# liuQuan98/APR

Hardware: AMD Instinct MI355X
Metric: point-cloud pairs/sec (120k-pt KITTI frame, FCGF encode+match+SVD) (higher is better)
Workload: dtype f32

## Files before the change

apr_amd/_lib.py:

```python
from __future__ import annotations

import ctypes as C
import os

import torch

_HERE = os.path.dirname(os.path.abspath(__file__))
LIB_PATH = os.path.join(_HERE, "lib", "libapr_hip.so")

_p = C.c_void_p
_i32, _i64, _u64, _f32, _f64, _sz = C.c_int32, C.c_int64, C.c_uint64, C.c_float, C.c_double, C.c_size_t

class PairDesc(C.Structure):
    _fields_ = [("f0", C.c_void_p), ("n0", C.c_int64), ("f1", C.c_void_p), ("n1", C.c_int64),
                ("xyz0", C.c_void_p), ("xyz1", C.c_void_p), ("seed", C.c_uint64)]


class SpconvDesc(C.Structure):
    _fields_ = [("inp", C.c_void_p), ("ldi", C.c_int64), ("nbr", C.c_void_p), ("n_out", C.c_int64),
                ("K", C.c_int32), ("cin", C.c_int32), ("cout", C.c_int32), ("relu", C.c_int32),
                ("w_packed", C.c_void_p), ("scale", C.c_void_p), ("shift", C.c_void_p),
                ("residual", C.c_void_p), ("ldr", C.c_int64), ("out", C.c_void_p), ("ldo", C.c_int64),
                ("counters", C.c_void_p), ("plist", C.c_void_p), ("prod_scratch", C.c_void_p),
                ("plist_bytes", C.c_int64), ("w_bf3", C.c_void_p),
# ... 99 lines not shown
    "apr_norm_backward_scratch_bytes": (_sz, [_i64, _i32]),
    "apr_norm_backward": (C.c_int, [_p, _i64, _p, _i64, _i64, _i32, _p, _p, _p, _p, _i64, _p, _p, _p, _sz, _p]),
    "apr_bn_train_fwd": (C.c_int, [_p, _i64, _i64, _i32, _p, _p, C.c_float, C.c_float, _p, _p, _p, _i64, _i32, _p, _i64, _p, _p,
                                   _p, _p, _i32, _p, _sz, _p]),
    "apr_bn_train_bwd": (C.c_int, [_p, _i64, _p, _i64, _p, _i64, _i64, _i32, _p, _p, _p, _i32, _p, _i64, _p, _i64, _p, _p,
                                   _p, _i32, _p, _sz, _p]),
    "apr_weights_flip_transpose": (C.c_int, [_p, _i32, _i32, _i32, _i32, _p, _p]),
    "apr_dense_gemm_bf3": (C.c_int, [_p, _i64, _i64, _i32, _i32, _p, _p, _p, _p, _i64, _i32, _p, _i64, _p]),
    "apr_dense_rows_bf3_ok": (_i32, [_i32, _i32]),
    "apr_dense_rows_bf3_route": (_i32, [_i64, _i32, _i32]),
    "apr_dense_rows_bf3": (C.c_int, [_p, _i64, _i64, _i32, _i32, _p, _p, _p, _p, _i64, _i32, _i32, _p, _i64, _p]),
    "apr_dense_gemm_bf3_norm_scratch_bytes": (_sz, [_i64, _i32, _i32]),
    "apr_dense_gemm_bf3_norm_act": (C.c_int, [_p, _i64, _i64, _i32, _i32, _p, _f32, _p, _i64, _i32, _f32, _p, _i64, _p, _i32, _p,
                                              _sz, _p]),
    "apr_weighted_choice_round": (C.c_int64, [_p, _i64, _p, _i64, _i64, _p, _i64, _p, _p, _i32]),
    "apr_instance_norm_act_seg": (C.c_int, [_p, _i64, _i64, _i32, _f32, _p, _i64, _i32, _f32, _p, _i64, _p, _i32, _p, _sz, _p]),
    "apr_affine_act": (C.c_int, [_p, _i64, _i64, _i32, _p, _p, _p, _i64, _i32, _f32, _p, _i64, _p]),
    "apr_act_backward": (C.c_int, [_p, _i64, _p, _i64, _i64, _i32, _i32, _f32, _p, _i64, _p]),
    "apr_l2_normalize": (C.c_int, [_p, _i64, _i64, _i32, _p, _i64, _p]),
    "apr_l2_normalize_backward": (C.c_int, [_p, _i64, _p, _i64, _i64, _i32, _p, _i64, _p]),
    "apr_feature_nn": (C.c_int, [_p, _i64, _p, _i64, _i32, _p, _p]),
    "apr_feature_nn_fast_scratch_bytes": (_sz, [_i64, _i64, _i32]),
    "apr_feature_nn_fast": (C.c_int, [_p, _i64, _p, _i64, _i32, _p, _p, _sz, _p]),
    "apr_nn_unpack": (C.c_int, [_p, _i64, _p, _p, _p]),
    "apr_ransac_scratch_bytes": (_sz, [_i64, _i64]),
    "apr_ransac_pose": (C.c_int, [_p, _i64, _p, _i64, _p, _f64, _f64, _i64, _u64, _p, _sz, _p, _p]),
    "apr_ransac_geometric_scratch_bytes": (_sz, [_i64, _i64, _i64]),
    "apr_ransac_pose_geometric": (C.c_int, [_p, _i64, _p, _i64, _p, _f64, _f64, _i64, _i64, _u64, _p, _sz, _p, _p]),
    "apr_ransac_raw_bytes": (_sz, []),
    "apr_ransac_pose_geometric_async": (C.c_int, [_p, _i64, _p, _i64, _p, _f64, _f64, _i64, _i64, _u64, _p, _sz, _p, _p]),
    "apr_ransac_decode": (C.c_int, [_p, _p]),
    "apr_irls_pose": (C.c_int, [_p, _p, _p, _i64, _p, _p, _sz, _p]),
    "apr_match_pose_batch_scratch_bytes": (_sz, [_i32, _i64, _i64, _i32, _i64]),
    "apr_match_pose_batch": (C.c_int, [_p, _i32, _i32, C.c_double, C.c_double, _i64, _p, _sz, _p, _p]),
    "apr_match_pose_batch_slot_bytes": (_sz, [_i32]),
    "apr_match_pose_set_lanes": (C.c_int, [_i32]),
    "apr_match_pose_batch_enqueue": (C.c_int, [_p, _i32, _i32, C.c_double, C.c_double, _i64, _p, _sz, _p, _p]),
    "apr_match_pose_batch_finish": (C.c_int, [_p, _i32, _i32, C.c_double, C.c_double, _i64, _p, _sz, _p, _p, _p]),
    "apr_irls_scratch_bytes": (_sz, [_i64]),
    "apr_valid_pair": (C.c_int, [_p, _i64, _p, _i64, _p, _p, _i64, _i64, _p, _p, _f32, _p, _i64, _i64, _p, _sz, _p]),
    "apr_valid_pair_scratch_bytes": (_sz, [_i64]),
    "apr_contrastive_reduce": (C.c_int, [_p, _p, _i32, _i32, _p, _p, _p, _p, _p, _p, _p, _i32, _i64, _f32, _f32, _p, _p]),
    "apr_grid_subsample_scratch_bytes": (_sz, [_i64]),
    "apr_grid_subsample": (C.c_int, [_p, _i64, _p, _i32, _f32, _p, _i32, _p, _p, _p, _p, _sz, _p]),
    "apr_grid_subsample_async": (C.c_int, [_p, _i64, _p, _i32, _f32, _p, _i32, _p, _p, _p, _p, _sz, _p]),
    "apr_voxel_down_sample_scratch_bytes": (_sz, [_i64]),
# ... 130 lines not shown
```

apr_amd/csrc/common.h:

```cpp
#pragma once
#include <hip/hip_runtime.h>
#include <stdint.h>
#include <stdio.h>
#include <stdlib.h>
#include <string.h>

#include "../../include/apr_hip.h"

static inline int env_int(const char* name, int dflt) {
  const char* v = getenv(name);
  return v ? atoi(v) : dflt;
}

#define APR_API extern "C" __attribute__((visibility("default")))

void apr_set_error(const char* fmt, ...);

#define APR_CHECK_ARG(cond, ...)      \
  do {                                \
    if (!(cond)) {                    \
      apr_set_error(__VA_ARGS__);     \
      return APR_EINVAL;              \
    }                                 \
  } while (0)
// ... 9 lines not shown

#define APR_LAUNCH_CHECK() APR_HIP(hipGetLastError())

static inline int64_t cdiv64(int64_t a, int64_t b) { return (a + b - 1) / b; }

__host__ __device__ static inline size_t apr_align256(size_t x) { return (x + 255) & ~(size_t)255; }

struct AprArena {
  char* base;
  size_t off = 0;
  explicit AprArena(void* scratch) : base((char*)apr_align256((size_t)scratch)) {}
  template <typename T>
  T* take(size_t count) {
    T* p = base ? (T*)(base + off) : nullptr;
    off += apr_align256(count * sizeof(T));
    return p;
  }
  size_t bytes() const { return off + 256; }
  bool fits(size_t scratch_bytes) const { return scratch_bytes >= bytes(); }
};

int apr_internal_nn_brute(const float* f0, int64_t n0, const float* f1, int64_t n1, int32_t c, uint64_t* best,
                          const unsigned* run_if, void* stream);

int apr_internal_fill(void* ptr, int32_t byte_value, size_t bytes, hipStream_t st);

bool apr_internal_dense_ok(int64_t M, int32_t cin, int32_t cout);
bool apr_internal_dense_rows_route(int64_t M, int32_t cin, int32_t cout);
int apr_internal_dense_gemm(const float* in, int64_t ldi, int64_t M, int32_t cin, int32_t cout, const float* wp,
                            const float* scale, const float* shift, const float* residual, int64_t ldr, int32_t relu,
                            float* out, int64_t ldo, hipStream_t st);

int apr_internal_norm_apply_partials(const float* x, int64_t ldx, int32_t c, const int64_t* seg_row0, const int* seg_blk0,
                                     int32_t nseg, const double* partial, float eps, const float* residual, int64_t ldr,
                                     int32_t act_mode, float negative_slope, float* y, int64_t ldy, hipStream_t st);

#ifdef __HIPCC__
__device__ inline int apr_wave_incl_scan(int x) {
  x += __builtin_amdgcn_update_dpp(0, x, 0x111, 0xf, 0xf, true);
  x += __builtin_amdgcn_update_dpp(0, x, 0x112, 0xf, 0xf, true);
  x += __builtin_amdgcn_update_dpp(0, x, 0x114, 0xf, 0xf, true);
  x += __builtin_amdgcn_update_dpp(0, x, 0x118, 0xf, 0xf, true);
  x += __builtin_amdgcn_update_dpp(0, x, 0x142, 0xa, 0xf, true);
  x += __builtin_amdgcn_update_dpp(0, x, 0x143, 0xc, 0xf, true);
  return x;
}
// ... 83 lines not shown
```

apr_amd/csrc/match_mfma.hip:

```cpp
#include "common.h"

namespace {

typedef float f32x4 __attribute__((ext_vector_type(4)));
typedef float f32x2 __attribute__((ext_vector_type(2)));
typedef __bf16 bf16x8 __attribute__((ext_vector_type(8)));

constexpr float kEpsRel = 1e-4f;
constexpr float kEpsAbs = 5e-5f;

__device__ inline unsigned short to_bf16_rne(float x) {
  unsigned u = __float_as_uint(x);
  u += 0x7FFFu + ((u >> 16) & 1u);
  return (unsigned short)(u >> 16);
}

template <int C>
__global__ void k_nn_prep(const float* __restrict__ f, int64_t n, float len_scale, float row_scale,
                          unsigned short* __restrict__ fb, unsigned short* __restrict__ fl, f32x4* __restrict__ meta,
                          unsigned* __restrict__ u_init, unsigned long long* __restrict__ best_init,
                          unsigned* __restrict__ zero_me) {
  constexpr int LPR = C / 4;
  const int64_t t = (int64_t)blockIdx.x * blockDim.x + threadIdx.x;
  const int64_t row = t / LPR;
// ... 506 lines not shown
  const unsigned shared_cap = (unsigned)shared_capacity(n0);
  constexpr int LPR = C / 4;
  if ((uint64_t)qblocks * 4 * (uint64_t)nchunk * (uint64_t)(chunk / 16) + 64 >= (1ull << 32)) {
    apr_set_error("apr_feature_nn_fast: problem too large for the dense-block ids");
    return APR_EINVAL;
  }
  hipLaunchKernelGGL((k_nn_prep2<C>), dim3((unsigned)cdiv64((n0 + n1) * LPR, 256)), dim3(256), 0, st, f0, n0, f1, n1, qb, ql,
                     qmeta, tb, tl, tmeta, U, best, overflow);
  static const int s_dense_min = env_int("APR_NN_DENSE_MIN", kDenseMin);
  static const int s_bound_div = env_int("APR_NN_BOUND_DIV", 4);
  const dim3 grid((unsigned)qblocks, (unsigned)nchunk);
  hipLaunchKernelGGL((k_nn_mfma<C, false>), grid, dim3(256), 0, st, qb, ql, qmeta, n0, tb, tl, tmeta, n1, (int)chunk, U,
                     cand, cand_count, overflow, shared_list, shared_cap, dense_list, overflow + 2, s_bound_div);
  hipLaunchKernelGGL((k_nn_mfma<C, true>), grid, dim3(256), 0, st, qb, ql, qmeta, n0, tb, tl, tmeta, n1, (int)chunk, U,
                     cand, cand_count, overflow, shared_list, shared_cap, dense_list, overflow + 2, s_dense_min);
  const unsigned nwg = (unsigned)(qblocks * nchunk);
  const unsigned nexact = nwg + 256;
  hipLaunchKernelGGL((k_nn_resolve<C>), dim3(nexact + 1024), dim3(256), 0, st, cand, cand_count, nwg, nexact, shared_list,
                     overflow, shared_cap, dense_list, (int)chunk, (unsigned)(qblocks * 4), f0, n0, f1, n1, best);
  APR_LAUNCH_CHECK();
  return APR_OK;
}

}

APR_API size_t apr_feature_nn_fast_scratch_bytes(int64_t n0, int64_t n1, int32_t c) {
  if (n0 < 0 || n1 < 0 || c <= 0) return 0;
  if (n0 < 1) n0 = 1;
  if (n1 < 1) n1 = 1;
  const size_t qblocks = (size_t)cdiv64(n0, 256);
  const size_t nwaves = 4 * (768 + qblocks);
  const size_t nflag = qblocks * 4 * ((2 * (size_t)n1 + 320) / 16 + 1);
  const size_t nlist = nflag > kDenseListCap ? (size_t)kDenseListCap : nflag;
  const auto al = apr_align256;
  return 2 * al((size_t)n0 * c * 2) + 2 * al((size_t)n1 * c * 2) + al((size_t)n0 * 16) + al((size_t)n1 * 16) +
         al((size_t)n0 * 4) + 256 + al(nwaves * 4) + al(nwaves * kCandWave * 8) +
         al((size_t)shared_capacity(n0) * 8) + al(nflag + 64) + al(nlist * 4 + 64) + 512;
}

APR_API int apr_feature_nn_fast(const float* f0, int64_t n0, const float* f1, int64_t n1, int32_t c, uint64_t* best,
                                void* scratch, size_t scratch_bytes, void* stream) {
  hipStream_t st = (hipStream_t)stream;
  APR_CHECK_ARG(n0 >= 0 && n1 > 0 && n1 < (1ll << 31) && n0 < (1ll << 31), "apr_feature_nn_fast: bad shape");
  APR_CHECK_ARG(c == 32 || c == 64 || c == 128, "apr_feature_nn_fast: c=%d, supported: 32, 64, 128", c);
  APR_CHECK_ARG(n1 < (1ll << 24) - 64, "apr_feature_nn_fast: n1 = %lld, supported below 2^24 - 64 targets", (long long)n1);
  APR_CHECK_ARG(((((uintptr_t)f0) | ((uintptr_t)f1)) & 15) == 0, "apr_feature_nn_fast: 16-byte aligned rows required");
  APR_CHECK_ARG(scratch_bytes >= apr_feature_nn_fast_scratch_bytes(n0, n1, c), "apr_feature_nn_fast: scratch too small");
  if (n0 == 0) return APR_OK;
  unsigned long long* b = (unsigned long long*)best;
  if (c == 32) return run_fast<32>(f0, n0, f1, n1, b, scratch, scratch_bytes, st);
  if (c == 64) return run_fast<64>(f0, n0, f1, n1, b, scratch, scratch_bytes, st);
  return run_fast<128>(f0, n0, f1, n1, b, scratch, scratch_bytes, st);
}
```

apr_amd/csrc/ransac.hip:

```cpp
#include <atomic>
#include <cstring>
#include <map>
#include <mutex>
#include <utility>

#include "common.h"
#include "irls.h"

namespace {

struct Hyp {
  double T[12];
  long long it;
  int inliers;
  int pad;
  double err2;
};

__host__ __device__ inline uint64_t splitmix64(uint64_t z) {
  z = (z ^ (z >> 30)) * 0xBF58476D1CE4E5B9ull;
  z = (z ^ (z >> 27)) * 0x94D049BB133111EBull;
  return z ^ (z >> 31);
}

__host__ __device__ inline uint32_t sample_index(uint64_t seed, uint64_t it, int slot, uint32_t n) {
  uint64_t z = splitmix64(seed + (it * 4ull + (uint64_t)slot + 1ull) * 0x9E3779B97F4A7C15ull);
  return (uint32_t)(((z >> 32) * (uint64_t)n) >> 32);
// ... 1371 lines not shown
APR_API size_t apr_match_pose_batch_slot_bytes(int32_t B) { return B > 0 ? (size_t)B * kSlotBytes : 0; }

APR_API int apr_match_pose_batch_enqueue(const apr_pair_desc* pairs, int32_t B, int32_t c, double max_dist,
                                         double edge_ratio, int64_t max_iter, void* scratch, size_t scratch_bytes,
                                         void* slots_host, void* stream) {
  hipStream_t st = (hipStream_t)stream;
  APR_CHECK_ARG(B > 0 && B <= 4096 && pairs && slots_host, "apr_match_pose_batch: bad arguments");
  APR_CHECK_ARG(max_iter > 0 && max_iter < (1ll << 31) && max_dist > 0 && c > 0, "apr_match_pose_batch: bad parameters");
  int64_t n0_max = 0, n1_max = 0;
  for (int i = 0; i < B; ++i) {
    APR_CHECK_ARG(pairs[i].n0 > 0 && pairs[i].n1 > 0 && pairs[i].n0 < (1ll << 31) && pairs[i].n1 < (1ll << 31),
                  "apr_match_pose_batch: empty point set in pair %d", i);
    n0_max = pairs[i].n0 > n0_max ? pairs[i].n0 : n0_max;
    n1_max = pairs[i].n1 > n1_max ? pairs[i].n1 : n1_max;
  }
  AprArena arena(scratch);
  const BatchScratch L = walk_batch(arena, scratch_bytes, B, n0_max, n1_max, c, max_iter);
  APR_CHECK_ARG(L.lanes >= 1, "apr_match_pose_batch: scratch too small");
  const int nlanes = L.lanes;
  char* const slots = L.slots;
  const int64_t cap = max_iter < kChunk ? max_iter : kChunk;
  const double thr_lt = sqrt_lt_threshold(max_dist);
  const bool fast_nn = (c == 32 || c == 64 || c == 128);
  hipStream_t lane_st[kMaxLanes] = {st};
  struct EventGuard {
    hipEvent_t e = nullptr;
    ~EventGuard() { if (e) (void)hipEventDestroy(e); }
  } fork;
  if (nlanes > 1) {
    SideStreams ss;
    const int rc = side_streams(st, &ss);
    if (rc != APR_OK) return rc;
    APR_HIP(hipEventCreateWithFlags(&fork.e, hipEventDisableTiming));
    APR_HIP(hipEventRecord(fork.e, st));
    for (int l = 1; l < nlanes; ++l) {
      lane_st[l] = ss.s[l - 1];
      APR_HIP(hipStreamWaitEvent(lane_st[l], fork.e, 0));
    }
  }
  int rc = APR_OK;
  for (int i = 0; i < B && rc == APR_OK; ++i) {
    const apr_pair_desc& d = pairs[i];
    const int l = i % nlanes;
    hipStream_t ls = lane_st[l];
    char* lp = L.lane0 + (size_t)l * L.lane_bytes;
    uint64_t* best = (uint64_t*)(lp + L.best_off);
    rc = fast_nn ? apr_feature_nn_fast(d.f0, d.n0, d.f1, d.n1, c, best, lp, L.nn_bytes, ls)
                 : apr_feature_nn(d.f0, d.n0, d.f1, d.n1, c, best, ls);
    if (rc != APR_OK) break;
    int64_t* corr = (int64_t*)(L.corr + (size_t)i * L.corr_each);
    AprArena ra(lp + L.ransac_off);
    RansacScratch r = walk_ransac(ra, d.n0, max_iter);
    r.best = (Hyp*)(slots + (size_t)i * kSlotBytes);
    r.total_valid = (long long*)((char*)r.best + sizeof(Hyp));
    hipLaunchKernelGGL(k_init_best, dim3(1), dim3(128), 0, ls, r.best, r.total_valid, r.maxn2, r.n_valid, counter_words(r));
    launch_pack(r, d.xyz0, d.xyz1, d.n1, (const int64_t*)best, d.n0, ls, corr);
    launch_hypotheses(r, d.n0, max_dist, edge_ratio, 0, max_iter, d.seed, (int)cap, ls, true);
    launch_scoring(r, d.n0, thr_lt, (int)cap, ls);
  }
  if (nlanes > 1) {
    for (int l = 1; l < nlanes; ++l) {
      EventGuard join;
      APR_HIP(hipEventCreateWithFlags(&join.e, hipEventDisableTiming));
      APR_HIP(hipEventRecord(join.e, lane_st[l]));
      APR_HIP(hipStreamWaitEvent(st, join.e, 0));
    }
  }
  if (rc != APR_OK) return rc;
  APR_LAUNCH_CHECK();
  APR_HIP(hipMemcpyAsync(slots_host, slots, (size_t)B * kSlotBytes, hipMemcpyDeviceToHost, st));
  return APR_OK;
// ... 186 lines not shown
```

apr_amd/ops.py:

```python
from __future__ import annotations

import ctypes as C
import os

import numpy as np
import torch

from . import _lib
from ._lib import check, ptr, stream


def _lib_():
    return _lib.load()


def _f32(t, name):
    if not t.is_cuda or t.dtype != torch.float32:
        raise _lib.AprHipError(f"{name}: need a float32 GPU tensor (no CPU fallback), got {t.dtype} on {t.device}")
    return t


def _rows(t, name):
    _f32(t, name)
    if t.dim() != 2 or (t.shape[1] > 1 and t.stride(1) != 1):
# ... 1030 lines not shown
    f1 = _f32(f1, "feature_nn.f1").contiguous()
    if f0.shape[1] != f1.shape[1]:
        raise _lib.AprHipError("feature_nn: channel mismatch")
    n0, c = f0.shape
    n1 = f1.shape[0]
    lib = _lib_()
    best = torch.empty(n0, dtype=torch.int64, device=f0.device)
    if impl is None:
        impl = os.environ.get("APR_NN_IMPL", "fast")
    if impl not in ("brute", "fast"):
        raise _lib.AprHipError(f"feature_nn: unknown impl {impl!r}")
    if impl == "fast" and c in (32, 64, 128):
        sb = int(lib.apr_feature_nn_fast_scratch_bytes(n0, n1, c))
        scratch = torch.empty(sb, dtype=torch.uint8, device=f0.device)
        check(lib.apr_feature_nn_fast(ptr(f0), n0, ptr(f1), n1, c, ptr(best), ptr(scratch), sb, stream()))
    else:
        check(lib.apr_feature_nn(ptr(f0), n0, ptr(f1), n1, c, ptr(best), stream()))
    idx = torch.empty(n0, dtype=torch.int64, device=f0.device)
    d2 = torch.empty(n0, dtype=torch.float32, device=f0.device) if return_distance else None
    check(lib.apr_nn_unpack(ptr(best), n0, ptr(idx), ptr(d2), stream()))
    return (idx, d2) if return_distance else idx



def _dev(t, dtype, name):
    if not torch.is_tensor(t) or not t.is_cuda or t.dtype != dtype:
        raise _lib.AprHipError(f"{name}: need a {dtype} GPU tensor (no CPU fallback), got "
                               f"{getattr(t, 'dtype', type(t))} on {getattr(t, 'device', 'the host')}")
    return t.contiguous()


def overlap_labels(correspondence, n_src, n_tgt):
    corr = _dev(correspondence, torch.int64, "overlap_labels.correspondence")
    dev = corr.device
    gt = torch.empty(n_src + n_tgt, dtype=torch.float32, device=dev)
    src_idx = torch.empty(n_src, dtype=torch.int32, device=dev)
    tgt_idx = torch.empty(n_tgt, dtype=torch.int32, device=dev)
    counts = torch.empty(3, dtype=torch.int32, device=dev)
    check(_lib_().apr_overlap_labels(ptr(corr), corr.shape[0], n_src, n_tgt, ptr(gt), ptr(src_idx), ptr(tgt_idx), ptr(counts),
                                     stream()))
    return gt, src_idx, tgt_idx, counts


def weighted_bce(pred, gt, n_dev=None):
    pred, gt = _dev(pred, torch.float32, "weighted_bce.pred"), _dev(gt, torch.float32, "weighted_bce.gt")
    if pred.dim() != 1 or pred.shape != gt.shape:
# ... 699 lines not shown
```

include/apr_hip.h:

```cpp
#ifndef APR_HIP_H
#define APR_HIP_H

#include <stddef.h>
#include <stdint.h>

#ifdef __cplusplus
extern "C" {
#endif

#define APR_OK 0
#define APR_EINVAL (-1)
#define APR_EHIP (-2)
#define APR_ETIMEOUT (-3)
#define APR_ERANGE (-3)

const char* apr_last_error(void);
int apr_version(void);
int apr_device_count(void);
int32_t apr_struct_sizes(int32_t* out, int32_t n);
int apr_event_wait(void* event, int32_t poll_us);
int apr_event_wait_timeout(void* event, int32_t poll_us, int64_t timeout_us);


int64_t apr_hash_capacity(int64_t n);
// ... 228 lines not shown
int apr_ransac_pose_geometric_async(const float* xyz0, int64_t n0, const float* xyz1, int64_t n1,
                                    const int64_t* corr, double max_dist, double edge_ratio, int64_t max_iter,
                                    int64_t max_validation, uint64_t seed, void* scratch, size_t scratch_bytes,
                                    void* raw_dev, void* stream);
int apr_ransac_decode(const void* raw_host, double* result_host);

typedef struct {
  const float* f0; int64_t n0;
  const float* f1; int64_t n1;
  const float* xyz0;
  const float* xyz1;
  uint64_t seed;
} apr_pair_desc;
size_t apr_match_pose_batch_scratch_bytes(int32_t B, int64_t n0_max, int64_t n1_max, int32_t c, int64_t max_iter);
int apr_match_pose_batch(const apr_pair_desc* pairs, int32_t B, int32_t c, double max_dist, double edge_ratio,
                         int64_t max_iter, void* scratch, size_t scratch_bytes, double* results_host, void* stream);
size_t apr_match_pose_batch_slot_bytes(int32_t B);
int apr_match_pose_batch_enqueue(const apr_pair_desc* pairs, int32_t B, int32_t c, double max_dist, double edge_ratio,
                                 int64_t max_iter, void* scratch, size_t scratch_bytes, void* slots_host, void* stream);
int apr_match_pose_batch_finish(const apr_pair_desc* pairs, int32_t B, int32_t c, double max_dist, double edge_ratio,
                                int64_t max_iter, void* scratch, size_t scratch_bytes, const void* slots_host,
                                double* results_host, void* stream);

int apr_ransac_set_screen(int32_t mode);
int apr_ransac_set_option(int32_t option, int32_t value);
int apr_ransac_sampling_launches(int64_t* out2);

int apr_match_pose_set_lanes(int32_t lanes);

int apr_irls_pose(const float* pts0, const float* pts1, const float* weight, int64_t n,
                  float* T_host, void* scratch, size_t scratch_bytes, void* stream);
size_t apr_irls_scratch_bytes(int64_t n);

#define APR_VALID_RECORD_FLOATS 24
int apr_valid_pair(const float* xyz0, int64_t n0, const float* xyz1, int64_t n1, const int64_t* sel0,
                   const int64_t* sel1, int64_t m0, int64_t m1, const int64_t* nn, const float* T_gt,
                   float hit_thresh, float* records, int64_t n_slots, int64_t slot, void* scratch,
                   size_t scratch_bytes, void* stream);
size_t apr_valid_pair_scratch_bytes(int64_t m0);

int apr_contrastive_reduce(const float* pos_f0, const float* pos_f1, int32_t p, int32_t c,
                           const uint64_t* nn01, const uint64_t* nn10, const int64_t* sel0, const int64_t* sel1,
                           const int64_t* pos_ind0, const int64_t* pos_ind1, const int64_t* sorted_pos_keys,
                           int32_t n_keys, int64_t hash_seed, float pos_thresh, float neg_thresh,
                           double* out6, void* stream);

// ... 244 lines not shown
```

Measured before the change: 2756.

## Batch feature nearest-neighbour search across pairs with a two-pass MFMA bound sweep

Adds a batched feature-NN path that packs up to eight pairs into single prep, sweep and resolve launches. The sweep runs a bound pass, then a refine pass that emits candidate lists, which are resolved exactly in fp32, with a brute-force fallback when the lists overflow. The match+pose batch uses this path when there are enough query blocks, instead of running one chunked NN call per pair on the lane streams. This aims to cut per-pair launch overhead and fill the GPU better, at the cost of more scratch memory and more complex overflow handling.

Result: slower. 2722 (-1.2%).

```diff
diff --git a/apr_amd/_lib.py b/apr_amd/_lib.py
--- a/apr_amd/_lib.py
+++ b/apr_amd/_lib.py
@@ -145,6 +145,10 @@
     "apr_feature_nn": (C.c_int, [_p, _i64, _p, _i64, _i32, _p, _p]),
     "apr_feature_nn_fast_scratch_bytes": (_sz, [_i64, _i64, _i32]),
     "apr_feature_nn_fast": (C.c_int, [_p, _i64, _p, _i64, _i32, _p, _p, _sz, _p]),
+    "apr_feature_nn_batch_scratch_bytes": (_sz, [_i32, _i64, _i64, _i32]),
+    "apr_feature_nn_batch_carve_bytes": (_sz, [_p, _i32, _i32]),
+    "apr_feature_nn_batch": (C.c_int, [_p, _i32, _i32, _p, _p, _sz, _p]),
+    "apr_nn_set_option": (C.c_int, [_i32, _i32]),
     "apr_nn_unpack": (C.c_int, [_p, _i64, _p, _p, _p]),
     "apr_ransac_scratch_bytes": (_sz, [_i64, _i64]),
     "apr_ransac_pose": (C.c_int, [_p, _i64, _p, _i64, _p, _f64, _f64, _i64, _u64, _p, _sz, _p, _p]),
diff --git a/apr_amd/csrc/common.h b/apr_amd/csrc/common.h
--- a/apr_amd/csrc/common.h
+++ b/apr_amd/csrc/common.h
@@ -55,6 +55,10 @@
 
 int apr_internal_nn_brute(const float* f0, int64_t n0, const float* f1, int64_t n1, int32_t c, uint64_t* best,
                           const unsigned* run_if, void* stream);
+
+bool apr_internal_nn_batch_wanted(const apr_pair_desc* pairs, int32_t B, int32_t c);
+int apr_internal_nn_sweep(const apr_pair_desc* pairs, int32_t B, int32_t c, uint64_t* const* best, void* scratch,
+                          size_t scratch_bytes, void* stream);
 
 int apr_internal_fill(void* ptr, int32_t byte_value, size_t bytes, hipStream_t st);
 
diff --git a/apr_amd/csrc/match_mfma.hip b/apr_amd/csrc/match_mfma.hip
--- a/apr_amd/csrc/match_mfma.hip
+++ b/apr_amd/csrc/match_mfma.hip
@@ -1,3 +1,5 @@
+#include <atomic>
+
 #include "common.h"
 
 namespace {
@@ -552,6 +554,545 @@
   return APR_OK;
 }
 
+
+constexpr int kNnMaxPairs = 8;
+constexpr int kSweepCandWave = 8192;
+constexpr int kResolveSplit = 4;
+constexpr int kResolveShared = 64;
+constexpr int kResolveDense = 256;
+
+struct NnPairSlot {
+  const float *f0, *f1;
+  unsigned short *qb, *ql, *tb, *tl;
+  f32x4 *qmeta, *tmeta;
+  unsigned* ctl;
+  unsigned* cand_count;
+  unsigned long long* cand;
+  unsigned long long* shared_list;
+  unsigned* dense_list;
+  unsigned long long* best;
+  int n0, n1;
+  unsigned shared_cap, dense_cap;
+  int chunk, bound_len;
+  int qb0, prep0, res0;
+};
+struct NnTable {
+  NnPairSlot p[kNnMaxPairs];
+  int npairs, cand_wave, dense_min;
+};
+
+template <int C>
+__global__ void k_nn_prep_b(NnTable tab) {
+  constexpr int LPR = C / 4;
+  int p = 0;
+  while (p + 1 < tab.npairs && (int)blockIdx.x >= tab.p[p + 1].prep0) ++p;
+  const NnPairSlot& s = tab.p[p];
+  const int64_t n0 = s.n0, n1 = s.n1;
+  const int64_t t = (int64_t)((int)blockIdx.x - s.prep0) * 256 + threadIdx.x;
+  const int64_t row_all = t / LPR;
+  const int g = (int)(t - row_all * LPR);
+  const bool is_q = row_all < n0;
+  const int64_t row = is_q ? row_all : row_all - n0;
+  const int64_t n = is_q ? n0 : n1;
+  const float* f = is_q ? s.f0 : s.f1;
+  const float row_scale = is_q ? -2.0f : 1.0f, len_scale = is_q ? kEpsRel : 1.0f;
+  unsigned short* fb = is_q ? s.qb : s.tb;
+  unsigned short* fl = is_q ? s.ql : s.tl;
+  f32x4* meta = is_q ? s.qmeta : s.tmeta;
+  float sq = 0.f;
+  if (row < n) {
+    f32x4 v = *reinterpret_cast<const f32x4*>(f + row * C + g * 4);
+    sq = v[0] * v[0] + v[1] * v[1] + v[2] * v[2] + v[3] * v[3];
+    v *= row_scale;
+    ushort4 o, ol;
+    o.x = to_bf16_rne(v[0]); o.y = to_bf16_rne(v[1]); o.z = to_bf16_rne(v[2]); o.w = to_bf16_rne(v[3]);
+    ol.x = to_bf16_rne(v[0] - __uint_as_float((unsigned)o.x << 16));
+    ol.y = to_bf16_rne(v[1] - __uint_as_float((unsigned)o.y << 16));
+    ol.z = to_bf16_rne(v[2] - __uint_as_float((unsigned)o.z << 16));
+    ol.w = to_bf16_rne(v[3] - __uint_as_float((unsigned)o.w << 16));
+    *reinterpret_cast<ushort4*>(fb + row * C + g * 4) = o;
+    *reinterpret_cast<ushort4*>(fl + row * C + g * 4) = ol;
+  }
+#pragma unroll
+  for (int d = 1; d < LPR; d <<= 1) sq += __shfl_xor(sq, d);
+  float tlen = 0.f;
+  if (row < n && g == 0) {
+    const float nn = sq;
+    const float sl = kEpsAbs * nn;
+    const float len = sqrtf(nn);
+    meta[row] = (f32x4){len_scale * len, nn + sl, nn - sl, 0.f};
+    if (is_q) s.best[row] = ~0ull; else tlen = len;
+  }
+#pragma unroll
+  for (int d = 32; d >= 1; d >>= 1) tlen = fmaxf(tlen, __shfl_xor(tlen, d));
+  if ((threadIdx.x & 63) == 0 && tlen > 0.f) atomicMax(&s.ctl[3], __float_as_uint(tlen));
+}
+
+struct SweepBound { static constexpr bool refine = false; };
+struct SweepRefine { static constexpr bool refine = true; };
+
+template <int C>
+__global__ __launch_bounds__(256, 2) void k_nn_sweep(NnTable tab) {
+  constexpr int KS = C / 32, QT = 4, TR = C >= 128 ? 32 : 64, NT = TR / 16;
+  constexpr int LPT = (TR * C * 2) / 16 / 256;
+  __shared__ __attribute__((aligned(16))) unsigned short s_h[2][TR * C];
+  __shared__ __attribute__((aligned(16))) unsigned short s_l[2][TR * C];
+  __shared__ f32x4 s_m[2][TR];
+  __shared__ unsigned s_cand[4 * kCandBuf];
+  __shared__ unsigned s_dl[4 * kDlBuf];
+  __shared__ unsigned s_dn[4], s_dbase;
+  int p = 0;
+  while (p + 1 < tab.npairs && (int)blockIdx.x >= tab.p[p + 1].qb0) ++p;
+  const NnPairSlot& s = tab.p[p];
+  const unsigned qblk = blockIdx.x - (unsigned)s.qb0;
+  const int64_t n0 = s.n0, n1 = s.n1;
+  const unsigned short* __restrict__ qb = s.qb;
+  const unsigned short* __restrict__ ql = s.ql;
+  const unsigned short* __restrict__ tb = s.tb;
+  const unsigned short* __restrict__ tl = s.tl;
+  const f32x4* __restrict__ qmeta = s.qmeta;
+  const f32x4* __restrict__ tmeta = s.tmeta;
+  unsigned* const ctl = s.ctl;
+  unsigned long long* const shared_list = s.shared_list;
+  unsigned* const dense_list = s.dense_list;
+  const unsigned shared_cap = s.shared_cap, dense_cap = s.dense_cap;
+  const unsigned cand_wave = (unsigned)tab.cand_wave;
+  const int dense_min = tab.dense_min;
+  const unsigned ntiles = (unsigned)((n1 + 15) >> 4);
+  const int tid = threadIdx.x, lane = tid & 63, wave = tid >> 6;
+  const int l16 = lane & 15, lq = lane >> 4;
+  const int64_t q0 = (int64_t)qblk * 256 + wave * 64;
+  const bool wave_live = q0 < n0;
+  const unsigned wave_id = qblk * 4 + wave;
+  unsigned long long* const my_region = s.cand + (size_t)wave_id * cand_wave;
+  const float len_max = __uint_as_float(ctl[3]);
+  bf16x8 a[QT][KS], al[QT][KS];
+  float thr[QT][4], mn[QT][4];
+#pragma unroll
+  for (int qt = 0; qt < QT; ++qt) {
+    int64_t ra = q0 + qt * 16 + l16;
+    if (ra >= n0) ra = n0 - 1;
+#pragma unroll
+    for (int ks = 0; ks < KS; ++ks) {
+      a[qt][ks] = *reinterpret_cast<const bf16x8*>(qb + ra * C + ks * 32 + lq * 8);
+      al[qt][ks] = *reinterpret_cast<const bf16x8*>(ql + ra * C + ks * 32 + lq * 8);
+    }
+#pragma unroll
+    for (int r = 0; r < 4; ++r) {
+      mn[qt][r] = __builtin_inff();
+      thr[qt][r] = -__builtin_inff();
+    }
+  }
+  int ncand = 0, ndl = 0;
+  unsigned* my_dl = s_dl + wave * kDlBuf;
+  unsigned* my_cand = s_cand + wave * kCandBuf;
+  unsigned flushed = 0;
+
+  auto flush = [&]() {
+    if (ncand == 0) return;
+    auto entry = [&](int e) {
+      const unsigned c = my_cand[e];
+      return ((unsigned long long)(qblk * 256u + (c >> 24)) << 32) | (unsigned long long)(c & 0xffffffu);
+    };
+    if (flushed + ncand <= cand_wave) {
+      unsigned long long* dst = my_region + flushed;
+      for (int e = lane; e < ncand; e += 64) dst[e] = entry(e);
+      flushed += ncand;
+    } else {
+      unsigned base = 0;
+      if (lane == 0) base = atomicAdd(&ctl[1], (unsigned)ncand);
+      base = __shfl(base, 0);
+      if (base + (unsigned)ncand <= shared_cap) {
+        for (int e = lane; e < ncand; e += 64) shared_list[base + e] = entry(e);
+      } else if (lane == 0) {
+        ctl[0] = 1u;
+      }
+    }
+    ncand = 0;
+  };
+
+  uint4 rh[LPT], rl[LPT];
+  f32x4 rm;
+  auto fetch = [&](int64_t jt) {
+#pragma unroll
+    for (int u = 0; u < LPT; ++u) {
+      const int e = u * 256 + tid;
+      int64_t j = jt + (e * 8) / C;
+      if (j >= n1) j = n1 - 1;
+      const int64_t off = j * C + (e * 8) % C;
+      rh[u] = *reinterpret_cast<const uint4*>(tb + off);
+      rl[u] = *reinterpret_cast<const uint4*>(tl + off);
+    }
+    if (tid < TR) {
+      const int64_t j = jt + tid;
+      rm = tmeta[j < n1 ? j : n1 - 1];
+      if (j >= n1) {
+        rm[1] = __builtin_inff();
+        rm[2] = __builtin_inff();
+      }
+    }
+  };
+  auto commit = [&](int buf) {
+#pragma unroll
+    for (int u = 0; u < LPT; ++u) {
+      const int e = u * 256 + tid;
+      const int row = (e * 8) / C, kc = ((e * 8) % C) / 8;
+      const int at = (((kc >> 2) * TR + row) * 4 + (kc & 3)) * 8;
+      *reinterpret_cast<uint4*>(&s_h[buf][at]) = rh[u];
+      *reinterpret_cast<uint4*>(&s_l[buf][at]) = rl[u];
+    }
+    if (tid < TR) s_m[buf][tid] = rm;
+  };
+
+  auto sweep = [&](auto mode, int64_t chunk, int64_t blen) {
+    constexpr bool REFINE = decltype(mode)::refine;
+    int64_t c0 = 0, jt = 0;
+    fetch(0);
+    commit(0);
+    __builtin_amdgcn_s_waitcnt(0x0f70);
+    __syncthreads();
+    int buf = 0;
+    while (true) {
+      int64_t nj = jt + TR, nc0 = c0;
+      if (nj >= min((long long)(c0 + blen), (long long)n1)) {
+        nc0 = c0 + chunk;
+        nj = nc0;
+      }
+      const bool more = nj < n1;
+      if (more) fetch(nj);
+      if (wave_live) {
+        constexpr int NS = C >= 128 ? 1 : 2;
+        bf16x8 b[NS][KS], bl[NS][KS];
+        f32x4 tm[NS];
+        auto frag = [&](int slot, int tt) {
+#pragma unroll
+          for (int ks = 0; ks < KS; ++ks) {
+            b[slot][ks] = *reinterpret_cast<const bf16x8*>(&s_h[buf][((ks * TR + tt * 16 + l16) * 4 + lq) * 8]);
+            bl[slot][ks] = *reinterpret_cast<const bf16x8*>(&s_l[buf][((ks * TR + tt * 16 + l16) * 4 + lq) * 8]);
+          }
+          tm[slot] = s_m[buf][tt * 16 + l16];
+        };
+        frag(0, 0);
+#pragma unroll NS == 2 ? NT : 1
+        for (int tt = 0; tt < NT; ++tt) {
+          if (jt + tt * 16 >= n1) break;
+          const int cur = NS == 2 ? (tt & 1) : 0;
+          if (NS == 2 && tt + 1 < NT) frag(cur ^ 1, tt + 1);
+          if (NS == 1 && tt > 0) frag(0, tt);
+          const float cc = REFINE ? tm[cur][2] : tm[cur][1];
+          const f32x4 cinit = {cc, cc, cc, cc};
+          f32x4 acc[QT];
+#pragma unroll
+          for (int qt = 0; qt < QT; ++qt)
+            acc[qt] = __builtin_amdgcn_mfma_f32_16x16x32_bf16(al[qt][0], b[cur][0], cinit, 0, 0, 0);
+#pragma unroll
+          for (int qt = 0; qt < QT; ++qt)
+            acc[qt] = __builtin_amdgcn_mfma_f32_16x16x32_bf16(a[qt][0], bl[cur][0], acc[qt], 0, 0, 0);
+#pragma unroll
+          for (int ks = 1; ks < KS; ++ks) {
+#pragma unroll
+            for (int qt = 0; qt < QT; ++qt)
+              acc[qt] = __builtin_amdgcn_mfma_f32_16x16x32_bf16(al[qt][ks], b[cur][ks], acc[qt], 0, 0, 0);
+#pragma unroll
+            for (int qt = 0; qt < QT; ++qt)
+              acc[qt] = __builtin_amdgcn_mfma_f32_16x16x32_bf16(a[qt][ks], bl[cur][ks], acc[qt], 0, 0, 0);
+          }
+#pragma unroll
+          for (int ks = 0; ks < KS; ++ks)
+#pragma unroll
+            for (int qt = 0; qt < QT; ++qt)
+              acc[qt] = __builtin_amdgcn_mfma_f32_16x16x32_bf16(a[qt][ks], b[cur][ks], acc[qt], 0, 0, 0);
+          if (!REFINE) {
+#pragma unroll
+            for (int qt = 0; qt < QT; ++qt)
+#pragma unroll
+              for (int r = 0; r < 4; ++r)
+                mn[qt][r] = acc[qt][r] < mn[qt][r] ? acc[qt][r] : mn[qt][r];
+          } else {
+            unsigned cmask = 0;
+#pragma unroll
+            for (int qt = 0; qt < QT; ++qt)
+#pragma unroll
+              for (int r = 0; r < 4; ++r)
+                if (acc[qt][r] <= thr[qt][r]) cmask |= 1u << (qt * 4 + r);
+            if (__any(cmask != 0)) {
+              if (ncand > kCandBuf - 1024) flush();
+              const int c = __popc(cmask);
+              const int incl = apr_wave_incl_scan(c);
+              const int total = __builtin_amdgcn_readlane(incl, 63);
+              if (total >= dense_min) {
+                if (ndl == kDlBuf) {
+                  unsigned base = 0;
+                  if (lane == 0) base = atomicAdd(&ctl[2], (unsigned)ndl);
+                  base = __builtin_amdgcn_readfirstlane(base);
+                  for (int e = lane; e < ndl; e += 64) {
+                    if (base + e < dense_cap) dense_list[base + e] = my_dl[e]; else ctl[0] = 1u;
+                  }
+                  ndl = 0;
+                }
+                if (lane == 0) my_dl[ndl] = wave_id * ntiles + (unsigned)(jt >> 4) + tt;
+                ++ndl;
+                continue;
+              }
+              int pos = ncand + incl - c;
+              const unsigned j = (unsigned)jt + tt * 16 + l16;
+              while (cmask) {
+                const int e = __ffs((int)cmask) - 1;
+                cmask &= cmask - 1;
+                const unsigned i = wave * 64 + (e >> 2) * 16 + lq * 4 + (e & 3);
+                my_cand[pos++] = (i << 24) | j;
+              }
+              ncand += total;
+            }
+          }
+        }
+      }
+      if (more) commit(buf ^ 1);
+      __syncthreads();
+      if (!more) break;
+      jt = nj;
+      c0 = nc0;
+      buf ^= 1;
+    }
+  };
+
+  sweep(SweepBound{}, (int64_t)s.chunk, (int64_t)s.bound_len);
+#pragma unroll
+  for (int qt = 0; qt < QT; ++qt)
+#pragma unroll
+    for (int r = 0; r < 4; ++r) {
+      float v = mn[qt][r];
+#pragma unroll
+      for (int d = 1; d < 16; d <<= 1) v = fminf(v, __shfl_xor(v, d));
+      const int64_t row = q0 + qt * 16 + lq * 4 + r;
+      const bool live = row < n0;
+      const f32x4 m = qmeta[live ? row : n0 - 1];
+      const float u = fmaxf(v + m[1] + m[0] * len_max, 0.f);
+      thr[qt][r] = live ? u - m[2] + m[0] * len_max : -__builtin_inff();
+    }
+  sweep(SweepRefine{}, (int64_t)1 << 40, (int64_t)1 << 40);
+
+  flush();
+  if (lane == 0) {
+    s.cand_count[wave_id] = flushed;
+    s_dn[wave] = (unsigned)ndl;
+  }
+  __syncthreads();
+  if (tid == 0) {
+    const unsigned total = s_dn[0] + s_dn[1] + s_dn[2] + s_dn[3];
+    s_dbase = total ? atomicAdd(&ctl[2], total) : 0u;
+  }
+  __syncthreads();
+  unsigned base = s_dbase;
+  for (int w = 0; w < wave; ++w) base += s_dn[w];
+  for (int e = lane; e < ndl; e += 64) {
+    if (base + e < dense_cap) dense_list[base + e] = my_dl[e]; else ctl[0] = 1u;
+  }
+}
+
+template <int C>
+__global__ __launch_bounds__(256) void k_nn_resolve_b(NnTable tab, int nblocks) {
+  __shared__ __attribute__((aligned(16))) float s_t[4][16 * C];
+  int p = 0;
+  while (p + 1 < tab.npairs && (int)blockIdx.x >= tab.p[p + 1].res0) ++p;
+  const NnPairSlot& s = tab.p[p];
+  const unsigned lb = blockIdx.x - (unsigned)s.res0;
+  const unsigned pair_blocks = (unsigned)((p + 1 < tab.npairs ? tab.p[p + 1].res0 : nblocks) - s.res0);
+  const int64_t n0 = s.n0, n1 = s.n1;
+  const float* __restrict__ f0 = s.f0;
+  const float* __restrict__ f1 = s.f1;
+  unsigned long long* __restrict__ best = s.best;
+  const unsigned* ctl = s.ctl;
+  const int lane = threadIdx.x & 63;
+  const int wave = __builtin_amdgcn_readfirstlane(threadIdx.x >> 6);
+  const unsigned qwaves = (unsigned)((n0 + 255) >> 8) * 4u;
+  if (ctl[0] != 0u) {
+    const int64_t nqt = (n0 + 63) >> 6, ntt = (n1 + 15) >> 4;
+    const int64_t nw = (int64_t)pair_blocks * 4;
+    const int64_t slices = nw / nqt > 0 ? nw / nqt : 1;
+    const int64_t tps = (ntt + slices - 1) / slices;
+    for (int64_t w = (int64_t)lb * 4 + wave; w < nqt * slices; w += nw) {
+      const int64_t q = (w % nqt) * 64 + lane;
+      const int64_t tt0 = (w / nqt) * tps, tt1 = min((long long)(tt0 + tps), (long long)ntt);
+      const float* x = f0 + (q < n0 ? q : n0 - 1) * C;
+      f32x4 xv[C / 4];
+#pragma unroll
+      for (int g = 0; g < C / 4; ++g) xv[g] = *reinterpret_cast<const f32x4*>(x + g * 4);
+      float bd = __builtin_inff();
+      int bj = 0x7fffffff;
+      for (int64_t tt = tt0; tt < tt1; ++tt)
+        nn_tile_eval<C>(s_t[wave], xv, f1, tt * 16, min((long long)(tt * 16 + 16), (long long)n1), lane, bd, bj);
+      if (q < n0 && bj != 0x7fffffff) {
+        const unsigned long long mine = ((unsigned long long)__float_as_uint(bd) << 32) | (unsigned)bj;
+        if (mine < __builtin_nontemporal_load(&best[q])) atomicMin(&best[q], mine);
+      }
+    }
+    return;
+  }
+  const unsigned nregion = qwaves * kResolveSplit, nexact = nregion + kResolveShared;
+  if (lb < nexact) {
+    const bool shared = lb >= nregion;
+    const unsigned region = lb / kResolveSplit;
+    const unsigned n = shared ? min(ctl[1], s.shared_cap) : min(s.cand_count[region], (unsigned)tab.cand_wave);
+    const unsigned long long* src = shared ? s.shared_list : s.cand + (size_t)region * (unsigned)tab.cand_wave;
+    const unsigned first = (shared ? lb - nregion : lb % kResolveSplit) * 256u + threadIdx.x;
+    const unsigned step = (shared ? kResolveShared : kResolveSplit) * 256u;
+    for (unsigned t = first; t < n; t += step) {
+      const unsigned long long ij = src[t];
+      const int64_t i = (int64_t)(ij >> 32), j = (int64_t)(ij & 0xffffffffull);
+      const float* x = f0 + i * C;
+      const float* y = f1 + j * C;
+      float s0 = 0.f, s1 = 0.f, s2 = 0.f, s3 = 0.f;
+#pragma unroll
+      for (int g = 0; g < C / 4; ++g) {
+        const f32x4 xv = *reinterpret_cast<const f32x4*>(x + g * 4);
+        const f32x4 yv = *reinterpret_cast<const f32x4*>(y + g * 4);
+        const float d0 = xv[0] - yv[0], d1 = xv[1] - yv[1], d2 = xv[2] - yv[2], d3 = xv[3] - yv[3];
+        s0 = fmaf(d0, d0, s0);
+        s1 = fmaf(d1, d1, s1);
+        s2 = fmaf(d2, d2, s2);
+        s3 = fmaf(d3, d3, s3);
+      }
+      const float d = (s0 + s1) + (s2 + s3);
+      const unsigned long long mine = ((unsigned long long)__float_as_uint(d) << 32) | (unsigned)j;
+      if (mine < __builtin_nontemporal_load(&best[i])) atomicMin(&best[i], mine);
+    }
+    return;
+  }
+  const unsigned ntiles = (unsigned)((n1 + 15) >> 4);
+  const unsigned n = min(ctl[2], s.dense_cap);
+  const unsigned nwaves = (pair_blocks - nexact) * 4;
+  for (unsigned e = (lb - nexact) * 4 + wave; e < n; e += nwaves) {
+    const unsigned fb = __builtin_amdgcn_readfirstlane(s.dense_list[e]);
+    const unsigned wave_id = fb / ntiles, tile = fb % ntiles;
+    const int64_t q = (int64_t)wave_id * 64 + lane;
+    const int64_t j0 = (int64_t)tile * 16;
+    const int64_t j1 = min((long long)(j0 + 16), (long long)n1);
+    const float* x = f0 + (q < n0 ? q : n0 - 1) * C;
+    f32x4 xv[C / 4];
+#pragma unroll
+    for (int g = 0; g < C / 4; ++g) xv[g] = *reinterpret_cast<const f32x4*>(x + g * 4);
+    float bd = __builtin_inff();
+    int bj = 0x7fffffff;
+    nn_tile_eval<C>(s_t[wave], xv, f1, j0, j1, lane, bd, bj);
+    if (q < n0 && bj != 0x7fffffff) {
+      const unsigned long long mine = ((unsigned long long)__float_as_uint(bd) << 32) | (unsigned)bj;
+      if (mine < __builtin_nontemporal_load(&best[q])) atomicMin(&best[q], mine);
+    }
+  }
+}
+
+enum { kNnOptBatch = 0, kNnOptCandWave = 1, kNnOptDenseCap = 2, kNnOptN = 3 };
+std::atomic<int> g_nn_opt[kNnOptN] = {{-2}, {-2}, {-2}};
+
+int nn_option(int o) {
+  static const int s_env[kNnOptN] = {env_int("APR_NN_BATCH", -1), env_int("APR_NN_CAND_WAVE", 0),
+                                     env_int("APR_NN_DENSE_CAP", 0)};
+  const int v = g_nn_opt[o].load(std::memory_order_relaxed);
+  return v == -2 ? s_env[o] : v;
+}
+int sweep_cand_wave() {
+  const int v = nn_option(kNnOptCandWave);
+  return v > 0 && v < kSweepCandWave ? v : kSweepCandWave;
+}
+unsigned sweep_dense_cap() {
+  const int v = nn_option(kNnOptDenseCap);
+  return v > 0 && (unsigned)v < kDenseListCap ? (unsigned)v : kDenseListCap;
+}
+
+void walk_sweep_pair(AprArena& a, NnPairSlot* slot, int64_t n0, int64_t n1, int c, int cand_wave, unsigned dense_cap) {
+  const size_t qwaves = (size_t)cdiv64(n0, 256) * 4;
+  uint64_t ndense = (uint64_t)qwaves * (uint64_t)cdiv64(n1, 16);
+  if (ndense > dense_cap) ndense = dense_cap;
+  NnPairSlot t;
+  NnPairSlot& s = slot ? *slot : t;
+  s.qb = a.take<unsigned short>((size_t)n0 * c);
+  s.ql = a.take<unsigned short>((size_t)n0 * c);
+  s.tb = a.take<unsigned short>((size_t)n1 * c);
+  s.tl = a.take<unsigned short>((size_t)n1 * c);
+  s.qmeta = a.take<f32x4>(n0);
+  s.tmeta = a.take<f32x4>(n1);
+  s.cand_count = a.take<unsigned>(qwaves);
+  s.cand = a.take<unsigned long long>(qwaves * (size_t)cand_wave);
+  s.shared_list = a.take<unsigned long long>(shared_capacity(n0));
+  s.dense_list = a.take<unsigned>((size_t)ndense + 16);
+  s.shared_cap = (unsigned)shared_capacity(n0);
+  s.dense_cap = (unsigned)ndense;
+}
+
+template <int C>
+int run_sweep(const apr_pair_desc* pairs, int32_t B, uint64_t* const* best, void* scratch, size_t scratch_bytes,
+              hipStream_t st) {
+  static const int s_dense_min = env_int("APR_NN_DENSE_MIN", kDenseMin);
+  static const int s_bound_div = env_int("APR_NN_BOUND_DIV", 4);
+  const int cand_wave = sweep_cand_wave();
+  const unsigned dense_cap = sweep_dense_cap();
+  AprArena a(scratch);
+  unsigned* ctl = a.take<unsigned>((size_t)B * 64);
+  if ((size_t)B * 256 + 256 > scratch_bytes) {
+    apr_set_error("apr_feature_nn_batch: scratch too small");
+    return APR_EINVAL;
+  }
+  int rc = apr_internal_fill(ctl, 0, (size_t)B * 256, st);
+  if (rc != APR_OK) return rc;
+  constexpr int LPR = C / 4;
+  const int ngroups = (int)cdiv64(B, kNnMaxPairs), per = (int)cdiv64(B, ngroups);
+  for (int g0 = 0; g0 < B; g0 += per) {
+    NnTable tab;
+    memset(&tab, 0, sizeof(tab));
+    tab.cand_wave = cand_wave;
+    tab.dense_min = s_dense_min;
+    int np = 0, qb = 0, prep = 0, res = 0;
+    for (int i = g0; i < B && i < g0 + per; ++i) {
+      const apr_pair_desc& d = pairs[i];
+      if (d.n0 == 0) continue;
+      NnPairSlot& s = tab.p[np++];
+      walk_sweep_pair(a, &s, d.n0, d.n1, C, cand_wave, dense_cap);
+      s.f0 = d.f0;
+      s.f1 = d.f1;
+      s.n0 = (int)d.n0;
+      s.n1 = (int)d.n1;
+      s.ctl = ctl + (size_t)i * 64;
+      s.best = (unsigned long long*)best[i];
+      int64_t qblocks, chunk, nchunk;
+      nn_grid(d.n0, d.n1, C, &qblocks, &chunk, &nchunk);
+      s.chunk = (int)chunk;
+      s.bound_len = (int)((chunk / (s_bound_div > 0 ? s_bound_div : 1) + 63) / 64 * 64);
+      s.qb0 = qb;
+      s.prep0 = prep;
+      s.res0 = res;
+      qb += (int)qblocks;
+      prep += (int)cdiv64((d.n0 + d.n1) * LPR, 256);
+      res += (int)qblocks * 4 * kResolveSplit + kResolveShared + kResolveDense;
+    }
+    if (!a.fits(scratch_bytes)) {
+      apr_set_error("apr_feature_nn_batch: scratch too small");
+      return APR_EINVAL;
+    }
+    if (np == 0) continue;
+    tab.npairs = np;
+    hipLaunchKernelGGL((k_nn_prep_b<C>), dim3((unsigned)prep), dim3(256), 0, st, tab);
+    hipLaunchKernelGGL((k_nn_sweep<C>), dim3((unsigned)qb), dim3(256), 0, st, tab);
+    hipLaunchKernelGGL((k_nn_resolve_b<C>), dim3((unsigned)res), dim3(256), 0, st, tab, res);
+  }
+  APR_LAUNCH_CHECK();
+  return APR_OK;
+}
+
+int check_batch_args(const apr_pair_desc* pairs, int32_t B, int32_t c, const char* who) {
+  APR_CHECK_ARG(B > 0 && B <= 4096 && pairs, "%s: bad arguments", who);
+  APR_CHECK_ARG(c == 32 || c == 64 || c == 128, "%s: c=%d, supported: 32, 64, 128", who, c);
+  for (int i = 0; i < B; ++i) {
+    const apr_pair_desc& d = pairs[i];
+    APR_CHECK_ARG(d.n0 >= 0 && d.n1 > 0 && d.n0 < (1ll << 31), "%s: bad shape in pair %d", who, i);
+    APR_CHECK_ARG(d.n1 < (1ll << 24) - 64, "%s: n1 = %lld, supported below 2^24 - 64 targets", who, (long long)d.n1);
+    APR_CHECK_ARG(((((uintptr_t)d.f0) | ((uintptr_t)d.f1)) & 15) == 0, "%s: 16-byte aligned rows required", who);
+    APR_CHECK_ARG((uint64_t)cdiv64(d.n0, 256) * 4 * (uint64_t)cdiv64(d.n1, 16) < (1ull << 32),
+                  "%s: pair %d too large for the dense-block ids", who, i);
+  }
+  return APR_OK;
+}
+
 }
 
 APR_API size_t apr_feature_nn_fast_scratch_bytes(int64_t n0, int64_t n1, int32_t c) {
@@ -582,3 +1123,76 @@
   if (c == 64) return run_fast<64>(f0, n0, f1, n1, b, scratch, scratch_bytes, st);
   return run_fast<128>(f0, n0, f1, n1, b, scratch, scratch_bytes, st);
 }
+
+APR_API size_t apr_feature_nn_batch_carve_bytes(const apr_pair_desc* pairs, int32_t B, int32_t c) {
+  if (!pairs || B <= 0 || !(c == 32 || c == 64 || c == 128)) return 0;
+  AprArena a(nullptr);
+  a.take<unsigned>((size_t)B * 64);
+  const int cand_wave = sweep_cand_wave();
+  const unsigned dense_cap = sweep_dense_cap();
+  for (int i = 0; i < B; ++i) {
+    if (pairs[i].n0 < 0 || pairs[i].n1 <= 0) return 0;
+    if (pairs[i].n0 > 0) walk_sweep_pair(a, nullptr, pairs[i].n0, pairs[i].n1, c, cand_wave, dense_cap);
+  }
+  return a.bytes();
+}
+
+APR_API size_t apr_feature_nn_batch_scratch_bytes(int32_t B, int64_t n0_max, int64_t n1_max, int32_t c) {
+  if (B <= 0 || n0_max < 0 || n1_max < 0 || !(c == 32 || c == 64 || c == 128)) return 0;
+  if (n0_max < 1) n0_max = 1;
+  if (n1_max < 1) n1_max = 1;
+  AprArena a(nullptr);
+  a.take<unsigned>((size_t)B * 64);
+  for (int i = 0; i < B; ++i) walk_sweep_pair(a, nullptr, n0_max, n1_max, c, kSweepCandWave, kDenseListCap);
+  const size_t chunked = apr_feature_nn_fast_scratch_bytes(n0_max, n1_max, c);
+  return a.bytes() > chunked ? a.bytes() : chunked;
+}
+
+bool apr_internal_nn_batch_wanted(const apr_pair_desc* pairs, int32_t B, int32_t c) {
+  static const int s_min_qblocks = env_int("APR_NN_BATCH_MIN_QBLOCKS", 192);
+  const int mode = nn_option(kNnOptBatch);
+  if (mode == 0 || !(c == 32 || c == 64 || c == 128) || B <= 0) return false;
+  int64_t qblocks = 0;
+  for (int i = 0; i < B; ++i) {
+    if (pairs[i].n1 <= 0 || pairs[i].n1 >= (1ll << 24) - 64 || pairs[i].n0 < 0) return false;
+    qblocks += cdiv64(pairs[i].n0, 256);
+  }
+  if (qblocks == 0) return false;
+  return mode == 1 || qblocks / cdiv64(B, kNnMaxPairs) >= s_min_qblocks;
+}
+
+int apr_internal_nn_sweep(const apr_pair_desc* pairs, int32_t B, int32_t c, uint64_t* const* best, void* scratch,
+                          size_t scratch_bytes, void* stream) {
+  const int rc = check_batch_args(pairs, B, c, "apr_feature_nn_batch");
+  if (rc != APR_OK) return rc;
+  hipStream_t st = (hipStream_t)stream;
+  if (c == 32) return run_sweep<32>(pairs, B, best, scratch, scratch_bytes, st);
+  if (c == 64) return run_sweep<64>(pairs, B, best, scratch, scratch_bytes, st);
+  return run_sweep<128>(pairs, B, best, scratch, scratch_bytes, st);
+}
+
+APR_API int apr_feature_nn_batch(const apr_pair_desc* pairs, int32_t B, int32_t c, uint64_t* const* best, void* scratch,
+                                 size_t scratch_bytes, void* stream) {
+  const int rc = check_batch_args(pairs, B, c, "apr_feature_nn_batch");
+  if (rc != APR_OK) return rc;
+  APR_CHECK_ARG(best != nullptr, "apr_feature_nn_batch: NULL best");
+  if (apr_internal_nn_batch_wanted(pairs, B, c)) {
+    if (apr_feature_nn_batch_carve_bytes(pairs, B, c) <= scratch_bytes)
+      return apr_internal_nn_sweep(pairs, B, c, best, scratch, scratch_bytes, stream);
+    APR_CHECK_ARG(nn_option(kNnOptBatch) != 1, "apr_feature_nn_batch: scratch too small for the forced sweep form");
+  }
+  for (int i = 0; i < B; ++i) {
+    const int r = apr_feature_nn_fast(pairs[i].f0, pairs[i].n0, pairs[i].f1, pairs[i].n1, c, best[i], scratch,
+                                      scratch_bytes, stream);
+    if (r != APR_OK) return r;
+  }
+  return APR_OK;
+}
+
+APR_API int apr_nn_set_option(int32_t option, int32_t value) {
+  APR_CHECK_ARG(option >= 0 && option < kNnOptN, "apr_nn_set_option: option 0 .. 2");
+  APR_CHECK_ARG(option == kNnOptBatch ? (value >= -1 && value <= 1) : value >= -1,
+                "apr_nn_set_option: value out of range");
+  g_nn_opt[option].store(value == -1 ? -2 : value, std::memory_order_relaxed);
+  return APR_OK;
+}
diff --git a/apr_amd/csrc/ransac.hip b/apr_amd/csrc/ransac.hip
--- a/apr_amd/csrc/ransac.hip
+++ b/apr_amd/csrc/ransac.hip
@@ -3,6 +3,7 @@
 #include <map>
 #include <mutex>
 #include <utility>
+#include <vector>
 
 #include "common.h"
 #include "irls.h"
@@ -1420,6 +1421,24 @@
   const int64_t cap = max_iter < kChunk ? max_iter : kChunk;
   const double thr_lt = sqrt_lt_threshold(max_dist);
   const bool fast_nn = (c == 32 || c == 64 || c == 128);
+  const size_t best_each = apr_align256((size_t)n0_max * 8);
+  bool nn_batched = false;
+  if (fast_nn && apr_internal_nn_batch_wanted(pairs, B, c)) {
+    const size_t area = (size_t)nlanes * L.lane_bytes, bests = (size_t)B * best_each;
+    nn_batched = bests <= L.nn_bytes && apr_feature_nn_batch_carve_bytes(pairs, B, c) <= area - bests;
+    if (nn_batched) {
+      uint64_t* ptrs[64];
+      std::vector<uint64_t*> many;
+      uint64_t** bp = ptrs;
+      if (B > 64) {
+        many.resize(B);
+        bp = many.data();
+      }
+      for (int i = 0; i < B; ++i) bp[i] = (uint64_t*)(L.lane0 + (size_t)i * best_each);
+      const int rc_nn = apr_internal_nn_sweep(pairs, B, c, bp, L.lane0 + bests, area - bests, st);
+      if (rc_nn != APR_OK) return rc_nn;
+    }
+  }
   hipStream_t lane_st[kMaxLanes] = {st};
   struct EventGuard {
     hipEvent_t e = nullptr;
@@ -1442,9 +1461,10 @@
     const int l = i % nlanes;
     hipStream_t ls = lane_st[l];
     char* lp = L.lane0 + (size_t)l * L.lane_bytes;
-    uint64_t* best = (uint64_t*)(lp + L.best_off);
-    rc = fast_nn ? apr_feature_nn_fast(d.f0, d.n0, d.f1, d.n1, c, best, lp, L.nn_bytes, ls)
-                 : apr_feature_nn(d.f0, d.n0, d.f1, d.n1, c, best, ls);
+    uint64_t* best = nn_batched ? (uint64_t*)(L.lane0 + (size_t)i * best_each) : (uint64_t*)(lp + L.best_off);
+    if (!nn_batched)
+      rc = fast_nn ? apr_feature_nn_fast(d.f0, d.n0, d.f1, d.n1, c, best, lp, L.nn_bytes, ls)
+                   : apr_feature_nn(d.f0, d.n0, d.f1, d.n1, c, best, ls);
     if (rc != APR_OK) break;
     int64_t* corr = (int64_t*)(L.corr + (size_t)i * L.corr_each);
     AprArena ra(lp + L.ransac_off);
diff --git a/apr_amd/ops.py b/apr_amd/ops.py
--- a/apr_amd/ops.py
+++ b/apr_amd/ops.py
@@ -1076,6 +1076,51 @@
     return (idx, d2) if return_distance else idx
 
 
+def feature_nn_batch(feats0, feats1, return_distance=False):
+    B = len(feats0)
+    if B == 0 or B != len(feats1):
+        raise _lib.AprHipError("feature_nn_batch: need the same (non-zero) number of entries in both lists")
+    lib = _lib_()
+    descs = (_lib.PairDesc * B)()
+    keep, bests = [], []
+    c = feats0[0].shape[1]
+    n0m = n1m = 0
+    for i in range(B):
+        f0 = _f32(feats0[i], "feature_nn_batch.feats0").contiguous()
+        f1 = _f32(feats1[i], "feature_nn_batch.feats1").contiguous()
+        if f0.shape[1] != c or f1.shape[1] != c:
+            raise _lib.AprHipError("feature_nn_batch: channel mismatch in pair %d" % i)
+        keep += [f0, f1]
+        d = descs[i]
+        d.f0, d.n0, d.f1, d.n1 = f0.data_ptr(), f0.shape[0], f1.data_ptr(), f1.shape[0]
+        n0m, n1m = max(n0m, f0.shape[0]), max(n1m, f1.shape[0])
+        bests.append(torch.empty(f0.shape[0], dtype=torch.int64, device=f0.device))
+    sb = int(lib.apr_feature_nn_batch_scratch_bytes(B, n0m, n1m, c))
+    if sb == 0:
+        raise _lib.AprHipError("feature_nn_batch: C = %d, supported: 32, 64, 128" % c)
+    scratch = torch.empty(sb, dtype=torch.uint8, device=keep[0].device)
+    bp = (C.c_void_p * B)(*[b.data_ptr() for b in bests])
+    check(lib.apr_feature_nn_batch(descs, B, c, bp, ptr(scratch), sb, stream()))
+    out = []
+    for i in range(B):
+        n0 = descs[i].n0
+        idx = torch.empty(n0, dtype=torch.int64, device=bests[i].device)
+        d2 = torch.empty(n0, dtype=torch.float32, device=bests[i].device) if return_distance else None
+        if n0:
+            check(lib.apr_nn_unpack(ptr(bests[i]), n0, ptr(idx), ptr(d2), stream()))
+        out.append((idx, d2) if return_distance else idx)
+    return out
+
+
+def set_nn_batch(mode):
+    check(_lib_().apr_nn_set_option(0, -1 if mode is None else int(bool(mode))))
+
+
+def set_nn_caps(cand_wave=None, dense=None):
+    check(_lib_().apr_nn_set_option(1, -1 if cand_wave is None else int(cand_wave)))
+    check(_lib_().apr_nn_set_option(2, -1 if dense is None else int(dense)))
+
+
 
 def _dev(t, dtype, name):
     if not torch.is_tensor(t) or not t.is_cuda or t.dtype != dtype:
diff --git a/include/apr_hip.h b/include/apr_hip.h
--- a/include/apr_hip.h
+++ b/include/apr_hip.h
@@ -274,6 +274,12 @@
                                 int64_t max_iter, void* scratch, size_t scratch_bytes, const void* slots_host,
                                 double* results_host, void* stream);
 
+size_t apr_feature_nn_batch_scratch_bytes(int32_t B, int64_t n0_max, int64_t n1_max, int32_t c);
+size_t apr_feature_nn_batch_carve_bytes(const apr_pair_desc* pairs, int32_t B, int32_t c);
+int apr_feature_nn_batch(const apr_pair_desc* pairs, int32_t B, int32_t c, uint64_t* const* best, void* scratch,
+                         size_t scratch_bytes, void* stream);
+int apr_nn_set_option(int32_t option, int32_t value);
+
 int apr_ransac_set_screen(int32_t mode);
 int apr_ransac_set_option(int32_t option, int32_t value);
 int apr_ransac_sampling_launches(int64_t* out2);
```
